# tgm-team/tgm

Measured on AMD Instinct MI355X. Metric: sampled-edges/sec (TGAT 2-hop k=20 recency sampler, tgbl-wiki synthetic), higher is better.
Workload: dtype int32/int64 indices + f32 feature rows (copied, no arithmetic)

## Files before the change

include/tgm_amd.h:

```cpp
#ifndef TGM_AMD_H
#define TGM_AMD_H

#include <stddef.h>
#include <stdint.h>

#ifdef __cplusplus
extern "C" {
#endif

#define TGMX_ABI_VERSION 7

#define TGMX_OK 0
#define TGMX_E_INVALID (-1)
#define TGMX_E_LAUNCH (-2)
#define TGMX_E_UNSUPPORTED (-3)

#define TGMX_ST_SEED_RANGE 1
#define TGMX_ST_SEED_TIME 2
#define TGMX_ST_EDGE_RANGE 4
#define TGMX_ST_SCRATCH 8
#define TGMX_ST_TS_BOUND 16

typedef void* tgmx_stream_t;
typedef void* tgmx_event_t;
// ... 74 lines not shown
  int64_t n, eid0;
  int32_t directed, key_wrap32;
  int32_t* scratch;
  int32_t* status;
  int32_t timed_hop;
  tgmx_event_t ev_start, ev_stop;
  int64_t ts_bound;
  int32_t neg_group, neg_low, neg_high;
  uint64_t neg_seed, neg_call;
  int32_t* neg_out;
  int64_t* neg_time_out;
  int32_t guard_seed_errors;
  int32_t sorted_ts;
  int32_t* out_valid[TGMX_MAX_HOPS];
  int32_t* out_valid_prev[TGMX_MAX_HOPS];
  int64_t neg_index0;
  int64_t* csr_cursor;
  int32_t csr_x_by_pos;
  int32_t* out_eid[TGMX_MAX_HOPS];
  struct tgmx_defer* defer;
  int32_t defer_ok;
} tgmx_recency_step_t;

int tgmx_recency_step(const tgmx_recency_step_t* step, tgmx_stream_t stream);
int tgmx_recency_step_plan(const tgmx_recency_step_t* step);

typedef struct tgmx_defer tgmx_defer_t;
tgmx_defer_t* tgmx_defer_create(int32_t num_nodes, int32_t B);
void tgmx_defer_destroy(tgmx_defer_t* d);
int tgmx_defer_pending(const tgmx_defer_t* d);
int64_t tgmx_defer_count(const tgmx_defer_t* d);
int tgmx_defer_flush(tgmx_defer_t* d, tgmx_stream_t stream);
int32_t tgmx_set_fused_rows(int32_t rows);

#define TGMX_SEED_SRC 0
#define TGMX_SEED_DST 1
#define TGMX_SEED_NEG 2
typedef struct tgmx_pipeline {
  const int32_t* src;
  const int32_t* dst;
  const int64_t* ts;
  const float* edge_x;
  int64_t num_edges;
  int32_t rank, world;
  int32_t n_roles;
  int32_t seed_role[TGMX_MAX_SEED_GROUPS];
  int32_t neg_low, neg_high;
  uint64_t neg_seed;
  int32_t update;
  int32_t reserved0;
  tgmx_recency_step_t step;
} tgmx_pipeline_t;

typedef struct tgmx_pipeline_out {
  int32_t* neg;
  int64_t* neg_time;
  int32_t* seed_nid0;
  int64_t* seed_ts0;
  int32_t* out_nid[TGMX_MAX_HOPS];
  int64_t* out_ts[TGMX_MAX_HOPS];
  float* out_x[TGMX_MAX_HOPS];
  int32_t timed_hop;
  tgmx_event_t ev_start, ev_stop;
  int32_t* out_valid[TGMX_MAX_HOPS];
  int32_t* out_valid_prev[TGMX_MAX_HOPS];
  int32_t* out_eid[TGMX_MAX_HOPS];
// ... 505 lines not shown
```

tgm_amd/_native.py:

```python
from __future__ import annotations

import ctypes
import os
from ctypes import c_char_p, c_int32, c_int64, c_size_t, c_void_p
from typing import Optional

import torch

from .exceptions import NativeLibraryError

_HERE = os.path.dirname(os.path.abspath(__file__))
LIB_PATH = os.path.join(_HERE, 'csrc', 'libtgm_amd.so')

_P = c_void_p
SIGNATURES = {
    'tgmx_version': (c_int32, []),
    'tgmx_abi_sizeof': (c_size_t, [c_int32]),
    'tgmx_last_error': (c_char_p, []),
    'tgmx_event_create': (c_int32, [ctypes.POINTER(c_void_p)]),
    'tgmx_event_destroy': (c_int32, [_P]),
    'tgmx_event_elapsed_ms': (c_int32, [_P, _P, ctypes.POINTER(ctypes.c_float)]),
    'tgmx_recency_lookup_csr': (
        c_int32,
        [_P, _P, _P, c_int32, _P, _P, c_int64, c_int32, c_int32, c_int64, c_int64, c_int32, c_int32, _P, _P, _P, _P, _P, _P, _P],
# ... 263 lines not shown


class Pipeline(ctypes.Structure):

    _fields_ = [
        ('src', c_void_p), ('dst', c_void_p), ('ts', c_void_p), ('edge_x', c_void_p), ('num_edges', c_int64),
        ('rank', c_int32), ('world', c_int32), ('n_roles', c_int32), ('seed_role', c_int32 * MAX_SEED_GROUPS),
        ('neg_low', c_int32), ('neg_high', c_int32), ('neg_seed', ctypes.c_uint64),
        ('update', c_int32), ('reserved0', c_int32), ('step', RecencyStep),
    ]


class PipelineOut(ctypes.Structure):

    _fields_ = [
        ('neg', c_void_p), ('neg_time', c_void_p), ('seed_nid0', c_void_p), ('seed_ts0', c_void_p),
        ('out_nid', c_void_p * MAX_HOPS), ('out_ts', c_void_p * MAX_HOPS), ('out_x', c_void_p * MAX_HOPS),
        ('timed_hop', c_int32), ('ev_start', c_void_p), ('ev_stop', c_void_p),
        ('out_valid', c_void_p * MAX_HOPS), ('out_valid_prev', c_void_p * MAX_HOPS), ('out_eid', c_void_p * MAX_HOPS),
    ]


ACCOUNTING_PARTIALS = 1024
SIGNATURES['tgmx_lookup_accounting'] = (c_int32, [_P, c_int64, _P, _P, c_int64, _P, _P])
SIGNATURES['tgmx_uniform_lookup_csr'] = (c_int32, [_P, _P, _P, c_int32, _P, c_int64, c_int32, c_int64, c_int32, c_int32, ctypes.c_uint64, ctypes.c_uint64,
                                                   _P, _P, _P, _P, _P])
SIGNATURES['tgmx_ring_update_scratch_bytes'] = (c_size_t, [c_int64, c_int32])
SIGNATURES['tgmx_defer_create'] = (c_void_p, [c_int32, c_int32])
SIGNATURES['tgmx_defer_destroy'] = (None, [_P])
SIGNATURES['tgmx_defer_pending'] = (c_int32, [_P])
SIGNATURES['tgmx_defer_count'] = (c_int64, [_P])
SIGNATURES['tgmx_defer_flush'] = (c_int32, [_P, _P])
SIGNATURES['tgmx_set_fused_rows'] = (c_int32, [c_int32])
SIGNATURES['tgmx_tgn_gru_gate_backward'] = (c_int32, [_P, _P, _P, _P, c_int32, c_int64, _P, _P, _P])
SIGNATURES['tgmx_tgn_aggregate_backward'] = (c_int32, [c_int64, _P, _P, _P, _P, _P, _P, c_int32, c_int32, _P, _P, c_int32, c_int32, _P, _P, _P])
SIGNATURES['tgmx_tconv_edge_attr_backward'] = (c_int32, [_P, _P, _P, _P, _P, _P, c_int32, c_int32, c_int64, _P, _P])
SIGNATURES['tgmx_tconv_attend_backward'] = (c_int32, [_P, _P, _P, _P, _P, _P, _P, _P, c_int64, c_int32, c_int32, ctypes.c_float, _P, _P, _P, _P, _P, _P, _P])
SIGNATURES['tgmx_group_ids'] = (c_int32, [_P, c_int32, _P, _P, _P, _P, _P, _P])
SIGNATURES['tgmx_group_ids_workspace_bytes'] = (c_size_t, [c_int64])
SIGNATURES['tgmx_group_ids_large'] = (c_int32, [_P, c_int64, _P, _P, _P, _P, _P, _P, c_size_t, _P])
SIGNATURES['tgmx_random_negatives'] = (c_int32, [c_int32, c_int32, c_int64, ctypes.c_uint64, ctypes.c_uint64, _P, _P, c_int64, _P, _P])
SIGNATURES['tgmx_random_negatives_at'] = (c_int32, [c_int32, c_int32, c_int64, ctypes.c_uint64, ctypes.c_uint64, c_int64, _P, _P, c_int64, _P, _P])
SIGNATURES['tgmx_unique_ids_workspace_bytes'] = (c_size_t, [c_int32])
SIGNATURES['tgmx_unique_ids'] = (c_int32, [_P, _P, c_int32, c_int32, _P, _P, _P, _P, _P])
SIGNATURES['tgmx_csr_build_workspace_bytes'] = (c_size_t, [c_int64, c_int32, c_int32])
SIGNATURES['tgmx_csr_build'] = (c_int32, [_P, _P, _P, c_int64, c_int32, _P, c_int64, c_int32, _P, _P, _P, c_size_t, _P, _P])
SIGNATURES['tgmx_recency_step'] = (c_int32, [ctypes.POINTER(RecencyStep), _P])
SIGNATURES['tgmx_recency_step_plan'] = (c_int32, [ctypes.POINTER(RecencyStep)])
SIGNATURES['tgmx_pipeline_step'] = (c_int32, [ctypes.POINTER(Pipeline), c_int64, c_int64, ctypes.c_uint64, ctypes.POINTER(PipelineOut), ctypes.POINTER(PipelinePost), _P])
SIGNATURES['tgmx_event_synchronize'] = (c_int32, [_P])
SIGNATURES['tgmx_event_create_sync'] = (c_int32, [ctypes.POINTER(c_void_p)])
SIGNATURES['tgmx_event_record'] = (c_int32, [_P, _P])
SIGNATURES['tgmx_stream_wait_event'] = (c_int32, [_P, _P])
SIGNATURES['tgmx_stream_handoff'] = (c_int32, [_P, _P, _P])
SIGNATURES['tgmx_worker_create'] = (c_int32, [ctypes.POINTER(c_void_p)])
SIGNATURES['tgmx_worker_destroy'] = (c_int32, [_P])
SIGNATURES['tgmx_worker_pipeline_step'] = (c_int32, [_P, ctypes.POINTER(Pipeline), c_int64, c_int64, ctypes.c_uint64, ctypes.POINTER(PipelineOut),
                                                     ctypes.POINTER(PipelinePost), _P, _P, _P, ctypes.POINTER(ctypes.c_uint64)])
SIGNATURES['tgmx_worker_wait'] = (c_int32, [_P, ctypes.c_uint64])
SIGNATURES['tgmx_slice'] = (c_int32, [_P, c_int64, c_int32, c_int64, c_int32, c_int64, c_int64, c_int64, ctypes.POINTER(c_int64), ctypes.POINTER(c_int64)])
SIGNATURES['tgmx_discretize_workspace_bytes'] = (c_size_t, [c_int64])
SIGNATURES['tgmx_discretize_keep'] = (c_int32, [_P, _P, _P, c_int64, ctypes.c_double, _P, _P, _P, _P, c_size_t, _P])
SIGNATURES['tgmx_tgn_memory_forward'] = (c_int32, [ctypes.POINTER(TgnMemoryFwd), _P])
SIGNATURES['tgmx_tconv_forward'] = (c_int32, [ctypes.POINTER(TconvFwd), _P])
SIGNATURES['tgmx_tgn_step'] = (c_int32, [ctypes.POINTER(TgnStep), _P])
SIGNATURES['tgmx_segment_sort_workspace_bytes'] = (c_size_t, [c_int64])
# ... 184 lines not shown
```

tgm_amd/csrc/recency.hip:

```cpp
#include <algorithm>
#include <atomic>
#include <cstdlib>
#include <cstring>
#include <string>
#include <vector>

#include <hip/hip_ext.h>
#include <rocprim/block/block_radix_sort.hpp>
#include <rocprim/block/block_scan.hpp>
#include <rocprim/device/device_radix_sort.hpp>
#include <rocprim/device/device_scan.hpp>
#include <rocprim/iterator/counting_iterator.hpp>
#include <rocprim/iterator/transform_iterator.hpp>

#include "common.h"

namespace tgmx {

struct __align__(16) Rec {
  int nbr;
  int eid;
  long long ts;
};
static_assert(sizeof(Rec) == sizeof(tgmx_adj_t), "record layout");
// ... 220 lines not shown

__device__ __forceinline__ int logical_wp(const int32_t* write_pos, const unsigned long long* phdr, unsigned pstamp, int n) {
  const int wp = write_pos[n];
  const unsigned long long h = phdr ? phdr[n] : 0ull;
  return (phdr && (unsigned)(h >> 32) == pstamp) ? (int)(unsigned)h : wp;
}

__device__ __forceinline__ void publish_wp(const UpdateArgs& a, int n, int w0, int kept) {
  unsigned long long* hp = &a.dhdr[n];
  unsigned long long cur = __hip_atomic_load(hp, __ATOMIC_RELAXED, __HIP_MEMORY_SCOPE_AGENT);
  for (;;) {
    const int base = (unsigned)(cur >> 32) == a.dstamp ? (int)(unsigned)cur : w0;
    const unsigned long long nv = ((unsigned long long)a.dstamp << 32) | (unsigned)fold_add(base, kept, a.B);
    const unsigned long long prev = atomicCAS(hp, cur, nv);
    if (prev == cur) break;
    cur = prev;
  }
}

template <int MAXM>
struct PlaceLds {
  int sn[MAXM];
  int len[MAXM];
  int h_key[2 * MAXM], h_maxp[2 * MAXM];
  long long red[kBlockThreads / kWave], red2[kBlockThreads / kWave];
  int wave_tot[kBlockThreads / kWave];
};
template <int MAXM>
struct SortLds {
  long long key[MAXM];
  int pay[MAXM];
};

template <typename T>
__device__ __forceinline__ void st_agent(T* p, T v) {
  __hip_atomic_store(p, v, __ATOMIC_RELAXED, __HIP_MEMORY_SCOPE_AGENT);
}
template <typename T>
__device__ __forceinline__ T ld_agent(const T* p) {
  return __hip_atomic_load(p, __ATOMIC_RELAXED, __HIP_MEMORY_SCOPE_AGENT);
}

template <int E, int MAXM, bool PRESORTED, bool DEFER, bool COH = false>
__device__ __forceinline__ void update_block_body(const UpdateArgs& a, PlaceLds<MAXM>& L, SortLds<PRESORTED ? 1 : MAXM>& S,
                                                  int part = 0, int parts = 1) {
  constexpr int H = 2 * MAXM;
  constexpr int HBITS = MAXM == 512 ? 10 : (MAXM == 1024 ? 11 : (MAXM == 2048 ? 12 : 13));
  static_assert((1 << HBITS) == H, "hash size");
  long long* s_key = S.key;
  int* s_pay = S.pay;
  int* s_sn = L.sn;
  int* s_len = L.len;
  int* h_key = L.h_key;
  int* h_maxp = L.h_maxp;
  long long* red = L.red;
  long long* red2 = L.red2;
  int* wave_tot = L.wave_tot;
  const int m = (int)a.m;
  const int tid = threadIdx.x, lane = tid & 63, wave = tid >> 6;
  const int nthr = blockDim.x, nwaves = nthr >> 6;
  const int P = nthr * E;
  const bool blocked = DEFER ? false : update_blocked(a);

  for (int x = tid; x < H; x += nthr) {
    h_key[x] = -1;
    h_maxp[x] = -1;
  }
  int pay[E], node[E], w[E];
  if constexpr (PRESORTED) {
#pragma unroll
    for (int r = 0; r < E; ++r) {
      const int p = tid * E + r;
      pay[r] = p;
      node[r] = -1;
      w[r] = 0;
      if (p < m) {
        pay[r] = COH ? ld_agent(&a.sorted_j[p]) : a.sorted_j[p];
        node[r] = COH ? ld_agent(&a.sorted_node[p]) : a.sorted_node[p];
        w[r] = COH ? ld_agent(&a.target[p]) : a.target[p];
      }
    }
  } else {
    static_assert(PRESORTED || E == 1, "the in-kernel sort holds one element per thread");
    long long mx = strided_max_ts(a.ts, a.n, tid, nthr), mn = strided_min_ts(a.ts, a.n, tid, nthr);
    for (int off = 32; off > 0; off >>= 1) {
      const long long o = __shfl_xor(mx, off), o2 = __shfl_xor(mn, off);
      mx = o > mx ? o : mx;
      mn = o2 < mn ? o2 : mn;
    }
    if (lane == 0) {
      red[wave] = mx;
      red2[wave] = mn;
    }
    __syncthreads();
    mx = red[0];
    mn = red2[0];
    for (int wv = 1; wv < nwaves; ++wv) {
      mx = red[wv] > mx ? red[wv] : mx;
      mn = red2[wv] < mn ? red2[wv] : mn;
    }
    const long long span = mx + 1;
    const bool packed = can_pack(a.key_wrap32, mn, mx);
// ... 69 lines not shown
    hs[r] = 0;
    cnt[r] = 0;
    if (p < m && node[r] >= 0 && (parts == 1 || node[r] % parts == part)) {
      cnt[r] = s_len[st[r]];
      const int pos = p - st[r];
      const int drop = cnt[r] > a.B ? cnt[r] - a.B : 0;
      if (pos >= drop) {
        const int t = node[r] * a.B + (w[r] + pos - drop) % a.B;
        unsigned h = ((unsigned)t * 2654435761u) >> (32 - HBITS);
        for (;;) {
          const int old = atomicCAS(&h_key[h], -1, t);
          if (old == -1 || old == t) break;
          h = (h + 1) & (H - 1);
        }
        atomicMax(&h_maxp[h], p);
        tgt[r] = t;
        hs[r] = (int)h;
      }
    }
  }
  __syncthreads();

#pragma unroll
  for (int r = 0; r < E; ++r) {
    const int p = tid * E + r;
    if (p >= m) continue;
    if (parts > 1 && (node[r] >= 0 ? node[r] % parts : 0) != part) continue;
    int win = -1, kept = 0;
    if (tgt[r] >= 0) {
      if (h_maxp[hs[r]] == p) {
        Rec rec;
        if constexpr (DEFER) {
          if (a.drec) {
            const long long* src = reinterpret_cast<const long long*>(&a.sorted_rec[p]);
            long long* dst = reinterpret_cast<long long*>(&a.drec[tgt[r]]);
            dst[0] = COH ? ld_agent(&src[0]) : src[0];
            dst[1] = COH ? ld_agent(&src[1]) : src[1];
            a.dslot[tgt[r]] = (int32_t)a.dstamp;
          }
        } else if constexpr (PRESORTED) {
          rec = a.sorted_rec[p];
        } else {
          int nd, nbr;
          long long t, i;
          update_entry(a, pay[r], nd, nbr, t, i);
          rec.nbr = nbr;
          rec.eid = a.eid0 >= 0 ? (int)(a.eid0 + i) : -1;
          rec.ts = t;
        }
        if constexpr (!DEFER) {
          if (!blocked) a.ring[tgt[r]] = rec;
        }
        win = blocked ? -1 : tgt[r];
      }
      if (p == st[r] + cnt[r] - 1) {
        kept = cnt[r] > a.B ? a.B : cnt[r];
        if constexpr (!DEFER) {
          if (!blocked) commit_write_pos(&a.write_pos[node[r]], kept, a.B);
        } else {
          if (a.dhdr) publish_wp(a, node[r], w[r], kept);
        }
      }
    }
    a.winner[p] = win;
    if constexpr (DEFER) a.target[p] = kept;
    if constexpr (!PRESORTED) a.sorted_j[p] = pay[r];
  }
}

template <int E, int MAXM, bool PRESORTED>
__global__ __launch_bounds__(kBlockThreads) void ring_update_block_kernel(const UpdateArgs a) {
  __shared__ PlaceLds<MAXM> L;
  __shared__ SortLds<PRESORTED ? 1 : MAXM> S;
  update_block_body<E, MAXM, PRESORTED, false>(a, L, S, (int)blockIdx.x, (int)gridDim.x);
}

template <int E, int MAXM>
__global__ __launch_bounds__(kBlockThreads) void ring_update_decide_kernel(const UpdateArgs a) {
  __shared__ PlaceLds<MAXM> L;
  __shared__ SortLds<1> S;
  update_block_body<E, MAXM, true, true>(a, L, S, (int)blockIdx.x, (int)gridDim.x);
}


struct ChunkSortLds {
  long long key[kChunk];
  int pay[kChunk];
  long long red[kChunk / kWave], red2[kChunk / kWave];
};

template <bool AGENT = false>
__device__ __forceinline__ void update_chunk_sort(const UpdateArgs& a, int chunk, ChunkSortLds& W) {
  long long* s_key = W.key;
  int* s_pay = W.pay;
  long long* red = W.red;
  long long* red2 = W.red2;
  const int tid = threadIdx.x, lane = tid & 63, wave = tid >> 6;
  long long mx = strided_max_ts(a.ts, a.n, tid, kChunk), mn = strided_min_ts(a.ts, a.n, tid, kChunk);
  for (int off = 32; off > 0; off >>= 1) {
// ... 167 lines not shown
  bool valid[NE];
#pragma unroll
  for (int q = 0; q < NE; ++q) {
    valid[q] = act[q] && node[q] >= 0 && node[q] < a.N && nbr[q] >= 0 && nbr[q] < a.N;
    w[q] = valid[q] ? logical_wp(a.write_pos, a.phdr, a.pstamp, node[q]) : 0;
  }
#pragma unroll
  for (int q = 0; q < NE; ++q) {
    if (!act[q]) continue;
    int rank = tid;
#pragma unroll
    for (int o = 0; o < NC; ++o) rank += pos[q][o] >= 0 ? pos[q][o] : 0;
    if (!valid[q]) atomicOr(a.status, TGMX_ST_EDGE_RANGE);
    Rec rec;
    rec.nbr = nbr[q];
    rec.eid = a.eid0 >= 0 ? (int)(a.eid0 + i[q]) : -1;
    rec.ts = t[q];
    if constexpr (COH) {
      st_agent(&a.sorted_j[rank], pay[q]);
      st_agent(&a.sorted_node[rank], valid[q] ? node[q] : -1);
      st_agent(&a.target[rank], w[q]);
      long long* rd = reinterpret_cast<long long*>(&a.sorted_rec[rank]);
      st_agent(&rd[0], *reinterpret_cast<const long long*>(&rec));
      st_agent(&rd[1], rec.ts);
    } else {
      a.sorted_j[rank] = pay[q];
      a.sorted_node[rank] = valid[q] ? node[q] : -1;
      a.target[rank] = w[q];
      a.sorted_rec[rank] = rec;
    }
  }
}

constexpr int kSideSort = 1, kSideMerge = 2, kSidePlace = 3, kSideAll = 4, kSideSortMerge = 5, kSidePlaceOnly = 6, kSideSortMergePlace = 7, kSideMergePlace = 8;

__device__ __forceinline__ bool rider_barrier(int32_t* bar, int parts) {
  __syncthreads();
  bool ok = true;
  if (threadIdx.x == 0) {
    const int gen = __hip_atomic_load(&bar[1], __ATOMIC_RELAXED, __HIP_MEMORY_SCOPE_AGENT);
    const int prev = __hip_atomic_fetch_add(&bar[0], 1, __ATOMIC_RELAXED, __HIP_MEMORY_SCOPE_AGENT);
    if (prev == parts - 1) {
      __hip_atomic_store(&bar[0], 0, __ATOMIC_RELAXED, __HIP_MEMORY_SCOPE_AGENT);
      __builtin_amdgcn_s_waitcnt(0);
      __hip_atomic_fetch_add(&bar[1], 1, __ATOMIC_RELAXED, __HIP_MEMORY_SCOPE_AGENT);
    } else {
      int spins = 0;
      while (__hip_atomic_load(&bar[1], __ATOMIC_RELAXED, __HIP_MEMORY_SCOPE_AGENT) == gen) {
        __builtin_amdgcn_s_sleep(8);
        if (++spins > (1 << 19)) {
          ok = false;
          break;
        }
      }
    }
  }
  __syncthreads();
  return ok;
}
constexpr int kRidePlaceMaxM = 1024;

__device__ __forceinline__ void commit_position(const UpdateArgs& a, long long p) {
  const int row = a.winner[p];
  if (lane_id() == 0) {
    const int kept = a.target[p];
    if (row >= 0) a.ring[row] = a.sorted_rec[p];
    if (kept > 0) {
      const int n = a.sorted_node[p];
      if (a.dhdr) a.write_pos[n] = (int)(unsigned)a.dhdr[n];
      else commit_write_pos(&a.write_pos[n], kept, a.B);
    }
  }
  if (row < 0 || a.D == 0) return;
  const long long j = a.sorted_j[p];
  const long long i = j >= a.n ? j - a.n : j;
  float* __restrict__ o = a.ring_x + (long long)row * a.D;
  if (a.edge_x) {
    const float* __restrict__ x = a.edge_x + i * a.D;
    for (int c = lane_id(); c < a.D; c += kWave) o[c] = x[c];
  } else {
    for (int c = lane_id(); c < a.D; c += kWave) o[c] = 0.f;
  }
}

__device__ __forceinline__ void commit_block(const UpdateArgs& c, unsigned cb) {
  const long long p = (long long)cb * (blockDim.x >> 6) + (threadIdx.x >> 6);
  if (p < c.m) commit_position(c, p);
}

template <int PCAP>
union RiderLds {
  ChunkSortLds sort;
  SampleLds smp;
  PlaceLds<PCAP> place;
};
template <>
union RiderLds<0> {
  ChunkSortLds sort;
  SampleLds smp;
};

template <int PCAP = kRidePlaceMaxM>
__device__ __forceinline__ void update_side_work(const UpdateArgs& u, int stage, int block) {
  __shared__ RiderLds<PCAP> W;
  if (stage == kSideSort) {
    update_chunk_sort(u, block, W.sort);
  } else if (stage == kSideMerge) {
    update_merge_riding<1, kBlockMaxM / kChunk>(u, block, W.smp);
  } else if (stage == kSideSortMerge) {
    update_chunk_sort<true>(u, block, W.sort);
    if (!rider_barrier(u.barrier, (int)((u.m + kChunk - 1) / kChunk)) && threadIdx.x == 0) atomicOr(u.status, TGMX_ST_SCRATCH);
    update_merge_riding<1, kBlockMaxM / kChunk>(u, block, W.smp);
  } else if constexpr (PCAP > 0) {
    constexpr int NCH = PCAP / kChunk;
    if (stage == kSideSortMergePlace) {
      const int chunks = (int)((u.m + kChunk - 1) / kChunk);
      __shared__ int last_out;
      update_chunk_sort<true>(u, block, W.sort);
      if (!rider_barrier(u.barrier, chunks) && threadIdx.x == 0) atomicOr(u.status, TGMX_ST_SCRATCH);
      update_merge_riding<1, NCH, true>(u, block, W.smp);
      __syncthreads();
      if (threadIdx.x == 0) {
        const int prev = __hip_atomic_fetch_add(&u.barrier[5], 1, __ATOMIC_RELAXED, __HIP_MEMORY_SCOPE_AGENT);
        last_out = prev == chunks - 1;
        if (last_out) __hip_atomic_store(&u.barrier[5], 0, __ATOMIC_RELAXED, __HIP_MEMORY_SCOPE_AGENT);
      }
      __syncthreads();
      if (!last_out) return;
      SortLds<1> none;
      update_block_body<NCH, PCAP, true, true, true>(u, W.place, none);
      return;
    }
    if (stage == kSideMergePlace) {
      const int chunks = (int)((u.m + kChunk - 1) / kChunk);
      __shared__ int last_mp;
      update_merge_riding<1, NCH, true>(u, block, W.smp);
      __syncthreads();
      if (threadIdx.x == 0) {
        const int prev = __hip_atomic_fetch_add(&u.barrier[5], 1, __ATOMIC_RELAXED, __HIP_MEMORY_SCOPE_AGENT);
        last_mp = prev == chunks - 1;
        if (last_mp) __hip_atomic_store(&u.barrier[5], 0, __ATOMIC_RELAXED, __HIP_MEMORY_SCOPE_AGENT);
      }
      __syncthreads();
      if (!last_mp) return;
      SortLds<1> none;
      update_block_body<NCH, PCAP, true, true, true>(u, W.place, none);
      return;
    }
    if (stage == kSideAll) {
      const int chunks = (int)((u.m + kChunk - 1) / kChunk);
#pragma unroll 1
      for (int c = 0; c < NCH; ++c) {
        if (c < chunks) update_chunk_sort(u, c, W.sort);
        __syncthreads();
      }
    }
    if (stage != kSidePlaceOnly) {
      update_merge_riding<NCH, NCH>(u, 0, W.smp);
      __syncthreads();
    }
    SortLds<1> none;
    update_block_body<NCH, PCAP, true, true>(u, W.place, none);
  }
}


template <int GL>
__device__ __forceinline__ long long group_prefix_count(const Rec* recs, long long a, long long z, long long bound, int gl, int sub) {
  constexpr unsigned long long kMask = GL == 64 ? ~0ull : ((1ull << GL) - 1);
  long long lo = a, hi = z;
  while (__any(hi - lo > GL)) {
    const bool busy = hi - lo > GL;
    const long long len = hi - lo;
    const long long stride = (len + GL - 1) / GL;
    long long idx = lo + (long long)(gl + 1) * stride - 1;
    if (idx > hi - 1) idx = hi - 1;
    const bool less = busy && (long long)recs[idx].eid < bound;
    const int c = __popcll((__ballot(less) >> (sub * GL)) & kMask);
    if (busy) {
      long long nlo = lo, nhi = hi;
      if (c > 0) {
// ... 186 lines not shown
__device__ __forceinline__ void gather_rows(const LookupArgs& a, long long s, int k, int lane, const int* lds_eid, float* out_x, int first_slot) {
  using V = typename VecOf<VEC>::type;
  const V* __restrict__ X = reinterpret_cast<const V*>(a.edge_x);
  const int lim = a.pstore ? a.N * a.B : 0x7fffffff;
  const V* __restrict__ P = a.pstore ? reinterpret_cast<const V*>(a.pstore) : X;
  V* __restrict__ O = reinterpret_cast<V*>(out_x + s * (long long)k * a.D);
  const int total = k * a.row_vecs;
  constexpr int U = 8;
  for (int f0 = first_slot * a.row_vecs + lane; f0 < total; f0 += kWave * U) {
    const V* ptr[U];
    bool has[U];
#pragma unroll
    for (int u = 0; u < U; ++u) {
      const int f = f0 + u * kWave;
      const int fc = f < total ? f : f0;
      const int slot = (int)a.dv.div_nb((uint32_t)fc);
      const int col = fc - slot * a.row_vecs;
      const int e = lds_eid[slot];
      has[u] = e >= 0;
      const bool st = e >= lim;
      ptr[u] = (st ? P : X) + (has[u] ? (long long)(st ? e - lim : e) * a.row_vecs + col : 0);
    }
    V v[U];
#pragma unroll
    for (int u = 0; u < U; ++u) v[u] = *ptr[u];
#pragma unroll
    for (int u = 0; u < U; ++u) {
      const int f = f0 + u * kWave;
      if (f < total) O[f] = has[u] ? v[u] : zero_vec<V>();
    }
  }
}

template <bool RING, int VEC, bool SMALL>
__device__ __forceinline__ void lookup_seed(const LookupArgs& a, long long s, int n, long long q, int k, int lane, int* lds_eid,
                                            int32_t* out_nid, int64_t* out_ts, float* out_x, int32_t* out_valid, int32_t* out_valid_prev,
                                            int32_t* out_eid = nullptr) {
  const bool live = n >= 0 && n < a.N;
  int v_new = 0;
  if (SMALL) {
    const SmallPick o = small_pick<RING>(a, n, q, k, live, lane);
    if (lane < k) {
      out_nid[s * k + lane] = o.nbr;
      out_ts[s * k + lane] = o.ts;
      if (out_eid) out_eid[s * k + lane] = o.eid;
      lds_eid[lane] = o.src;
    }
    const unsigned long long m = __ballot(lane < k && o.has);
    v_new = m ? k - __builtin_ctzll(m) : 0;
  } else {
    const int B = a.B;
    const Window w = find_window<RING>(a, n, live, lane);
    int cnt = 0;
    for (int top = w.wlen; top > 0 && cnt == 0; top -= kWave) {
      const int lo = top > kWave ? top - kWave : 0;
      const int i = lo + lane;
      bool ok = false;
      if (i < top) {
        const Rec r = a.recs[slot_of<RING>(w, B, i)];
        ok = r.nbr >= 0 && r.ts < q;
      }
      const unsigned long long m = __ballot(ok);
      if (m) cnt = lo + 64 - __clzll((long long)m);
    }
    for (int c = lane; c < k; c += kWave) {
      const int i = cnt - k + c;
      Rec r;
      r.nbr = -1; r.eid = 0; r.ts = 0;
      if (i >= 0) r = a.recs[slot_of<RING>(w, B, i)];
      const bool has = r.nbr >= 0;
      out_nid[s * k + c] = has ? r.nbr : -1;
      out_ts[s * k + c] = has ? r.ts : 0;
      if (out_eid) out_eid[s * k + c] = has ? r.eid : -1;
      lds_eid[c] = has ? ((RING || a.x_by_pos) ? (int)slot_of<RING>(w, B, i) : r.eid) : -1;
      if (has && k - c > v_new) v_new = k - c;
    }
    for (int o = 32; o > 0; o >>= 1) {
      const int other = __shfl_xor(v_new, o);
      v_new = other > v_new ? other : v_new;
    }
  }
  if (a.D == 0 || out_x == nullptr) return;
  int first_slot = 0;
  if (out_valid) {
    const int v_old = out_valid[s];
    first_slot = k - (v_old > v_new ? v_old : v_new);
    if (lane == 0) {
      out_valid[s] = v_new;
      if (out_valid_prev) out_valid_prev[s] = v_old;
    }
  }
  __builtin_amdgcn_wave_barrier();
  gather_rows<VEC>(a, s, k, lane, lds_eid, out_x, first_slot);
  __builtin_amdgcn_wave_barrier();
}

template <bool RING, int VEC, bool SMALL, bool RIDE>
__global__ __launch_bounds__(256) void recency_lookup_kernel(const LookupArgs a, const UpdateArgs u) {
  extern __shared__ __attribute__((aligned(16))) int lds_eid_all[];
  unsigned bid = blockIdx.x, nblk = gridDim.x;
  if constexpr (RING && RIDE) {
    if (bid < a.side_blocks) {
      update_side_work(u, a.side_stage, (int)bid);
      return;
    }
    bid -= a.side_blocks;
    nblk -= a.side_blocks;
  }
  const int lane = lane_id();
  const int wave_in_block = threadIdx.x >> 6;
  int* lds_eid = lds_eid_all + wave_in_block * a.k;
  const long long waves_total = (long long)nblk * (blockDim.x >> 6);
  for (long long s = (long long)bid * (blockDim.x >> 6) + wave_in_block; s < a.S; s += waves_total) {
    int n;
    long long q;
    fetch_seed(a, s, lane, true, n, q);
    check_seed(a, n, q, a.allow_pad, lane);
    lookup_seed<RING, VEC, SMALL>(a, s, n, q, a.k, lane, lds_eid, a.out_nid, a.out_ts, a.out_x, a.out_valid, a.out_valid_prev, a.out_eid);
  }
}

constexpr int kFusedTsWords = 8;
constexpr int kFusedRowsDefault = 0;
enum FusedTsRole : long long { kTsRider = 1, kTsCommit = 2, kTsHop0 = 3, kTsHop1 = 4 };
__device__ __forceinline__ long long ts_after(int v) {
  asm volatile("" ::"v"(v));
  return (long long)wall_clock64();
}

template <bool RING>
__device__ __forceinline__ SmallPick fused_row_pick(const LookupArgs& a, const PickLoads& L, int n, long long q, bool live, int lane) {
  if constexpr (RING) return pick_finish(a, L, n, q, a.k1, live, lane);
  else return small_pick<false>(a, n, q, a.k1, live, lane);
}

template <bool RING, int VEC, int PCAP = kRidePlaceMaxM, bool ROWS = false, bool TS = false>
__global__ __launch_bounds__(256) void recency_lookup_fused01_kernel(const LookupArgs a, const UpdateArgs u, const UpdateArgs c) {
  extern __shared__ __attribute__((aligned(16))) int lds_eid_all[];
  unsigned bid = blockIdx.x, nblk = gridDim.x;
  const int lane = lane_id();
  const int wave_in_block = threadIdx.x >> 6;
  long long* ts_rec = TS ? a.ts + ((long long)blockIdx.x * (blockDim.x >> 6) + wave_in_block) * kFusedTsWords : nullptr;
  const long long t_start = TS ? (long long)wall_clock64() : 0;
  if constexpr (RING) {
    if (bid < a.side_blocks) {
      update_side_work<PCAP>(u, a.side_stage, (int)bid);
      if (TS && lane == 0) {
        ts_rec[0] = t_start;
        ts_rec[1] = (long long)wall_clock64();
        ts_rec[2] = kTsRider;
      }
      return;
    }
    bid -= a.side_blocks;
    if (bid < a.commit_blocks) {
      commit_block(c, bid);
      if (TS && lane == 0) {
        ts_rec[0] = t_start;
        ts_rec[1] = (long long)wall_clock64();
        ts_rec[2] = kTsCommit;
      }
      return;
    }
    bid -= a.commit_blocks;
    nblk -= a.side_blocks + a.commit_blocks;
  }
  const int k0 = a.k, k1 = a.k1;
  int* lds_eid = lds_eid_all + wave_in_block * (k0 > k1 ? k0 : k1);
  const long long waves_total = (long long)nblk * (blockDim.x >> 6);
  const long long S0 = a.S;
  const int G = ROWS ? a.fused_rows : 0;
  const int runs = G > 0 ? (k0 + G - 1) / G : k0;
  long long role = 0, t_seed = 0, t_index = 0, t_gather = 0;
  for (long long w = (long long)bid * (blockDim.x >> 6) + wave_in_block; w < S0 + S0 * runs; w += waves_total) {
    int n;
    long long q;
    if (w < S0) {
      role = kTsHop0;
      fetch_seed(a, w, lane, true, n, q);
      check_seed(a, n, q, 0, lane);
      lookup_seed<RING, VEC, true>(a, w, n, q, k0, lane, lds_eid, a.out_nid, a.out_ts, a.out_x, a.out_valid, a.out_valid_prev, a.out_eid);
    } else if (!ROWS) {
      role = kTsHop1;
      const long long idx = w - S0;
      const long long s0 = idx / k0;
      const int j = (int)(idx - s0 * k0);
      int n0;
      long long q0;
      fetch_seed(a, s0, lane, false, n0, q0);
      const SmallPick o = small_pick<RING>(a, n0, q0, k0, n0 >= 0 && n0 < a.N, lane);
      n = __shfl(o.nbr, j);
      q = __shfl(o.ts, j);
      lookup_seed<RING, VEC, true>(a, idx, n, q, k1, lane, lds_eid, a.out_nid1, a.out_ts1, a.out_x1, a.out_valid1, a.out_valid_prev1, a.out_eid1);
    } else {
      const long long run = w - S0;
      const long long s0 = run / runs;
      const int j0 = (int)(run - s0 * runs) * G;
      const int rows = k0 - j0 < G ? k0 - j0 : G;
      const long long base = s0 * k0 + j0;
      const bool feats = a.D > 0 && a.out_x1 != nullptr;
      const int v_old_run = (feats && a.out_valid1 && lane < rows) ? a.out_valid1[base + lane] : 0;
      int n0;
      long long q0;
      fetch_seed(a, s0, lane, false, n0, q0);
      const SmallPick o0 = small_pick<RING>(a, n0, q0, k0, n0 >= 0 && n0 < a.N, lane);
      n = __shfl(o0.nbr, j0);
      q = __shfl(o0.ts, j0);
      bool live = n >= 0 && n < a.N;
      if (TS) {
        role = kTsHop1 | ((long long)rows << 8);
        t_seed = ts_after(n);
      }
      PickLoads L = RING ? pick_issue(a, n, live, lane) : PickLoads{};
      for (int r = 0; r < rows; ++r) {
        const long long s = base + r;
        const long long t0 = TS ? (long long)wall_clock64() : 0;
        const SmallPick o = fused_row_pick<RING>(a, L, n, q, live, lane);
        if (lane < k1) {
          a.out_nid1[s * k1 + lane] = o.nbr;
          a.out_ts1[s * k1 + lane] = o.ts;
          if (a.out_eid1) a.out_eid1[s * k1 + lane] = o.eid;
          lds_eid[lane] = o.src;
        }
        const unsigned long long m = __ballot(lane < k1 && o.has);
        const int v_new = m ? k1 - __builtin_ctzll(m) : 0;
        if (TS) {
// ... 829 lines not shown
  static unsigned long long launches = 0;
  const long long waves = (long long)blocks_total * waves_per_block;
  std::vector<long long> h((size_t)(8 + waves * kFusedTsWords));
  if (hipStreamSynchronize(stream) != hipSuccess ||
      hipMemcpy(h.data() + 8, a.ts, (size_t)waves * kFusedTsWords * sizeof(long long), hipMemcpyDeviceToHost) != hipSuccess) {
    set_error("recency_lookup_fused01: reading the timestamps failed");
    return TGMX_E_LAUNCH;
  }
  int dev = 0, khz = 0;
  (void)hipGetDevice(&dev);
  (void)hipDeviceGetAttribute(&khz, hipDeviceAttributeWallClockRate, dev);
  const long long hdr[8] = {0x54474d5854530001ll, waves, (long long)a.side_blocks, (long long)a.commit_blocks, a.S, a.k, a.fused_rows, khz};
  std::copy(hdr, hdr + 8, h.begin());
  const std::string path = std::string(fused_ts_path()) + "." + std::to_string(launches++ % 16);
  if (FILE* f = fopen(path.c_str(), "wb")) {
    fwrite(h.data(), sizeof(long long), h.size(), f);
    fclose(f);
  }
  return TGMX_OK;
}

static std::atomic<int> g_fused_rows{-1};

static int fused_rows_per_wave(int k0) {
  int g = g_fused_rows.load(std::memory_order_relaxed);
  if (g < 0) {
    const char* e = getenv("TGMX_FUSED_ROWS");
    g = (e && *e && atoi(e) >= 0) ? atoi(e) : kFusedRowsDefault;
    g_fused_rows.store(g, std::memory_order_relaxed);
  }
  return g > k0 ? k0 : g;
}

template <bool RING>
static int launch_fused01(LookupArgs a, hipStream_t stream, hipEvent_t ev_start, hipEvent_t ev_stop, const UpdateArgs* side,
                          int side_stage, unsigned side_blocks, const UpdateArgs* commit = nullptr) {
  const UpdateArgs u = side ? *side : UpdateArgs{};
  const UpdateArgs c = (RING && commit) ? *commit : UpdateArgs{};
  a.side_blocks = (RING && side) ? side_blocks : 0;
  a.side_stage = side_stage;
  a.commit_blocks = (RING && commit) ? (unsigned)((c.m + 3) / 4) : 0u;
  a.fused_rows = fused_rows_per_wave(a.k);
  const int kmax = a.k > a.k1 ? a.k : a.k1;
  const int vec = prepare_lookup(a, a.out_x1, kmax);
  if (vec < 0) return vec;
  const int waves_per_block = 4;
  const long long runs = a.fused_rows > 0 ? (a.k + a.fused_rows - 1) / a.fused_rows : a.k;
  const long long waves = a.S + a.S * runs;
  long long blocks = (waves + waves_per_block - 1) / waves_per_block;
  if (blocks > (1 << 20)) blocks = 1 << 20;
  const dim3 grid((unsigned)blocks + a.side_blocks + a.commit_blocks), block(waves_per_block * kWave);
  const size_t lds = (size_t)waves_per_block * kmax * sizeof(int);
  const int pcap = !(RING && side) ? 1024 : ((side_stage != kSideAll && side_stage != kSideSortMergePlace) ? 0 : (u.m <= 512 ? 512 : 1024));
  if (RING && vec == 4 && pcap == 512 && fused_ts_path()) {
    static long long* ts_buf = nullptr;
    static size_t ts_cap = 0;
    const size_t need = (size_t)grid.x * waves_per_block * kFusedTsWords * sizeof(long long);
    if (need > ts_cap) {
      if (ts_buf) (void)hipFree(ts_buf);
      ts_buf = nullptr;
      if (hipMalloc(&ts_buf, need) != hipSuccess) {
        set_error("recency_lookup_fused01: no memory for the timestamps");
        return TGMX_E_LAUNCH;
      }
      ts_cap = need;
    }
    a.ts = ts_buf;
    (void)hipMemsetAsync(a.ts, 0, need, stream);
    if (a.fused_rows > 0) TGMX_LAUNCH_TIMED((recency_lookup_fused01_kernel<true, 4, 512, true, true>), grid, block, lds, stream, ev_start, ev_stop, a, u, c);
    else TGMX_LAUNCH_TIMED((recency_lookup_fused01_kernel<true, 4, 512, false, true>), grid, block, lds, stream, ev_start, ev_stop, a, u, c);
    TGMX_CHECK_LAUNCH("recency_lookup_fused01");
    return fused_ts_dump(a, stream, grid.x, waves_per_block);
  }
#define TGMX_FUSED(ROWS_)                                                                                                                            \
  do {                                                                                                                                               \
    if (vec == 4 && pcap == 512) TGMX_LAUNCH_TIMED((recency_lookup_fused01_kernel<RING, 4, RING ? 512 : 1024, ROWS_>), grid, block, lds, stream, ev_start, ev_stop, a, u, c); \
    else if (vec == 4 && pcap == 0) TGMX_LAUNCH_TIMED((recency_lookup_fused01_kernel<RING, 4, RING ? 0 : 1024, ROWS_>), grid, block, lds, stream, ev_start, ev_stop, a, u, c); \
    else if (vec == 4) TGMX_LAUNCH_TIMED((recency_lookup_fused01_kernel<RING, 4, kRidePlaceMaxM, ROWS_>), grid, block, lds, stream, ev_start, ev_stop, a, u, c);            \
    else if (vec == 2) TGMX_LAUNCH_TIMED((recency_lookup_fused01_kernel<RING, 2, kRidePlaceMaxM, ROWS_>), grid, block, lds, stream, ev_start, ev_stop, a, u, c);            \
    else TGMX_LAUNCH_TIMED((recency_lookup_fused01_kernel<RING, 1, kRidePlaceMaxM, ROWS_>), grid, block, lds, stream, ev_start, ev_stop, a, u, c);                          \
  } while (0)
  if (a.fused_rows > 0) TGMX_FUSED(true);
  else TGMX_FUSED(false);
#undef TGMX_FUSED
  TGMX_CHECK_LAUNCH("recency_lookup_fused01");
  return TGMX_OK;
// ... 719 lines not shown
}

extern "C" void tgmx_defer_destroy(tgmx_defer_t* d) {
  if (d && d->mem) (void)hipFree(d->mem);
  delete d;
}

static int defer_buffers(tgmx_defer* d, hipStream_t st) {
  if (d->mem) return TGMX_OK;
  auto up = [](size_t x) { return (x + 255) & ~(size_t)255; };
  const size_t nb = (size_t)d->N * d->B;
  const size_t half = up(tgmx_ring_update_scratch_bytes(kRidePlaceMaxM, 1));
  const size_t o_scr = up((size_t)16 * d->N), o_slot = o_scr + 2 * half, o_rec = up(o_slot + 8 * nb), total = o_rec + 32 * nb;
  void* mem = nullptr;
  if (hipMalloc(&mem, total) != hipSuccess) {
    set_error("recency_step: cannot allocate %zu bytes for the deferred commit", total);
    return TGMX_E_LAUNCH;
  }
  (void)hipMemsetAsync(mem, 0, o_rec, st);
  char* base = static_cast<char*>(mem);
  d->mem = mem;
  for (int q = 0; q < 2; ++q) {
    d->hdr[q] = reinterpret_cast<unsigned long long*>(base) + (size_t)q * d->N;
    d->scratch[q] = reinterpret_cast<int32_t*>(base + o_scr + q * half);
    d->slot[q] = reinterpret_cast<int32_t*>(base + o_slot) + q * nb;
    d->rec[q] = reinterpret_cast<Rec*>(base + o_rec) + q * nb;
  }
  return TGMX_OK;
}

extern "C" int tgmx_defer_pending(const tgmx_defer_t* d) { return d && d->pending ? 1 : 0; }

extern "C" int64_t tgmx_defer_count(const tgmx_defer_t* d) { return d ? d->deferred : 0; }
extern "C" int32_t tgmx_set_fused_rows(int32_t rows) {
  const int old = fused_rows_per_wave(1 << 30);
  g_fused_rows.store(rows < 0 ? -1 : rows, std::memory_order_relaxed);
  return old;
}

extern "C" int tgmx_defer_flush(tgmx_defer_t* d, tgmx_stream_t stream) {
  TGMX_REQUIRE(d, "defer_flush: null state");
  if (!d->pending) return TGMX_OK;
  d->pending = false;
  hipLaunchKernelGGL(ring_update_feat_kernel<true>, dim3((unsigned)((d->pend.m + 3) / 4)), dim3(256), 0, (hipStream_t)stream, d->pend);
  TGMX_CHECK_LAUNCH("defer_flush");
  return TGMX_OK;
}

static bool getenv_no_ride() {
  static const bool no_ride = getenv("TGMX_NO_RIDE") != nullptr;
  return no_ride;
}


static bool plan_fuse01(const tgmx_recency_step_t* s, long long S0) {
  static const bool no_fuse = getenv("TGMX_NO_FUSE") != nullptr;
  if (no_fuse || s->n_hops < 2 || S0 <= 0 || s->B > kWave || s->k[0] <= 0 || s->k[1] <= 0) return false;
  if (s->indptr != nullptr && (long long)s->k[1] * s->D * 4 < 4096) return false;
  static const bool fuse_by_id = !(getenv("TGMX_FUSE_BY_ID") && atoi(getenv("TGMX_FUSE_BY_ID")) == 0);
  const bool by_id = s->out_eid[1] != nullptr && s->out_x[1] == nullptr;
  if (s->indptr == nullptr && !(by_id && fuse_by_id)) {
    LookupArgs a{};
    a.B = s->B; a.D = s->D; a.edge_x = s->ring_x; a.out_x = s->out_x[0];
    if (prepare_lookup(a, s->out_x[1], s->k[1]) < 0) return false;
    if (packed_group_lanes(a, s->k[1], true) < 64) return false;
  }
// ... 221 lines not shown
```

Baseline: 9.458 billion.

## Add LDS-resident sort-and-place path for single rider block; hoist valid-span load

Adds a rider stage that sorts the update batch entirely in LDS (bitonic sort per chunk plus merge-rank across chunks) and feeds the deferred placement directly from LDS. This avoids writing and re-reading sorted records through global memory between stages. Separately, the old valid-span read is hoisted ahead of the seed fetch so its latency overlaps. The LDS path is gated by an env/setter flag that defaults off, so the default run only gets the hoisted load. The enlarged LDS union may reduce occupancy of the fused kernel.

Result: no change. 9.436 billion (-0.2%).

```diff
diff --git a/include/tgm_amd.h b/include/tgm_amd.h
--- a/include/tgm_amd.h
+++ b/include/tgm_amd.h
@@ -130,6 +130,7 @@
 int64_t tgmx_defer_count(const tgmx_defer_t* d);
 int tgmx_defer_flush(tgmx_defer_t* d, tgmx_stream_t stream);
 int32_t tgmx_set_fused_rows(int32_t rows);
+int32_t tgmx_set_rider_lds(int32_t on);
 
 #define TGMX_SEED_SRC 0
 #define TGMX_SEED_DST 1
diff --git a/tgm_amd/_native.py b/tgm_amd/_native.py
--- a/tgm_amd/_native.py
+++ b/tgm_amd/_native.py
@@ -319,6 +319,7 @@
 SIGNATURES['tgmx_defer_count'] = (c_int64, [_P])
 SIGNATURES['tgmx_defer_flush'] = (c_int32, [_P, _P])
 SIGNATURES['tgmx_set_fused_rows'] = (c_int32, [c_int32])
+SIGNATURES['tgmx_set_rider_lds'] = (c_int32, [c_int32])
 SIGNATURES['tgmx_tgn_gru_gate_backward'] = (c_int32, [_P, _P, _P, _P, c_int32, c_int64, _P, _P, _P])
 SIGNATURES['tgmx_tgn_aggregate_backward'] = (c_int32, [c_int64, _P, _P, _P, _P, _P, _P, c_int32, c_int32, _P, _P, c_int32, c_int32, _P, _P, _P])
 SIGNATURES['tgmx_tconv_edge_attr_backward'] = (c_int32, [_P, _P, _P, _P, _P, _P, c_int32, c_int32, c_int64, _P, _P])
diff --git a/tgm_amd/csrc/recency.hip b/tgm_amd/csrc/recency.hip
--- a/tgm_amd/csrc/recency.hip
+++ b/tgm_amd/csrc/recency.hip
@@ -276,6 +276,16 @@
   int pay[MAXM];
 };
 
+constexpr int kRiderLdsM = 2 * kChunk;
+struct SortedLds {
+  long long key[kRiderLdsM];
+  long long ts[kRiderLdsM];
+  int pay[kRiderLdsM];
+  int node[kRiderLdsM], nbr[kRiderLdsM];
+  int spay[kRiderLdsM];
+  long long red[kChunk / kWave], red2[kChunk / kWave];
+};
+
 template <typename T>
 __device__ __forceinline__ void st_agent(T* p, T v) {
   __hip_atomic_store(p, v, __ATOMIC_RELAXED, __HIP_MEMORY_SCOPE_AGENT);
@@ -285,9 +295,10 @@
   return __hip_atomic_load(p, __ATOMIC_RELAXED, __HIP_MEMORY_SCOPE_AGENT);
 }
 
-template <int E, int MAXM, bool PRESORTED, bool DEFER, bool COH = false>
+template <int E, int MAXM, bool PRESORTED, bool DEFER, bool COH = false, bool FROMLDS = false>
 __device__ __forceinline__ void update_block_body(const UpdateArgs& a, PlaceLds<MAXM>& L, SortLds<PRESORTED ? 1 : MAXM>& S,
-                                                  int part = 0, int parts = 1) {
+                                                  int part = 0, int parts = 1, const SortedLds* F = nullptr) {
+  static_assert(!FROMLDS || (PRESORTED && DEFER && !COH), "the LDS-fed placement is the deferred one of a single rider");
   constexpr int H = 2 * MAXM;
   constexpr int HBITS = MAXM == 512 ? 10 : (MAXM == 1024 ? 11 : (MAXM == 2048 ? 12 : 13));
   static_assert((1 << HBITS) == H, "hash size");
@@ -306,12 +317,37 @@
   const int P = nthr * E;
   const bool blocked = DEFER ? false : update_blocked(a);
 
+  int pay[E], node[E], w[E];
+  [[maybe_unused]] Rec lrec[FROMLDS ? E : 1];
+  if constexpr (FROMLDS) {
+#pragma unroll
+    for (int r = 0; r < E; ++r) {
+      const int p = tid * E + r;
+      pay[r] = p;
+      node[r] = -1;
+      w[r] = 0;
+      lrec[r].nbr = -1; lrec[r].eid = -1; lrec[r].ts = 0;
+      if (p < m) {
+        const int j = F->spay[p];
+        const int nd = F->node[j], nb = F->nbr[j];
+        const bool valid = nd >= 0 && nd < a.N && nb >= 0 && nb < a.N;
+        if (!valid) atomicOr(a.status, TGMX_ST_EDGE_RANGE);
+        pay[r] = j;
+        node[r] = valid ? nd : -1;
+        w[r] = valid ? logical_wp(a.write_pos, a.phdr, a.pstamp, nd) : 0;
+        lrec[r].nbr = nb;
+        lrec[r].eid = a.eid0 >= 0 ? (int)(a.eid0 + (j >= a.n ? j - a.n : j)) : -1;
+        lrec[r].ts = F->ts[j];
+      }
+    }
+    __syncthreads();
+  }
   for (int x = tid; x < H; x += nthr) {
     h_key[x] = -1;
     h_maxp[x] = -1;
   }
-  int pay[E], node[E], w[E];
-  if constexpr (PRESORTED) {
+  if constexpr (FROMLDS) {
+  } else if constexpr (PRESORTED) {
 #pragma unroll
     for (int r = 0; r < E; ++r) {
       const int p = tid * E + r;
@@ -447,10 +483,14 @@
         Rec rec;
         if constexpr (DEFER) {
           if (a.drec) {
-            const long long* src = reinterpret_cast<const long long*>(&a.sorted_rec[p]);
-            long long* dst = reinterpret_cast<long long*>(&a.drec[tgt[r]]);
-            dst[0] = COH ? ld_agent(&src[0]) : src[0];
-            dst[1] = COH ? ld_agent(&src[1]) : src[1];
+            if constexpr (FROMLDS) {
+              a.drec[tgt[r]] = lrec[r];
+            } else {
+              const long long* src = reinterpret_cast<const long long*>(&a.sorted_rec[p]);
+              long long* dst = reinterpret_cast<long long*>(&a.drec[tgt[r]]);
+              dst[0] = COH ? ld_agent(&src[0]) : src[0];
+              dst[1] = COH ? ld_agent(&src[1]) : src[1];
+            }
             a.dslot[tgt[r]] = (int32_t)a.dstamp;
           }
         } else if constexpr (PRESORTED) {
@@ -480,6 +520,11 @@
     a.winner[p] = win;
     if constexpr (DEFER) a.target[p] = kept;
     if constexpr (!PRESORTED) a.sorted_j[p] = pay[r];
+    if constexpr (FROMLDS) {
+      a.sorted_j[p] = pay[r];
+      a.sorted_node[p] = node[r];
+      a.sorted_rec[p] = lrec[r];
+    }
   }
 }
 
@@ -713,7 +758,89 @@
   }
 }
 
-constexpr int kSideSort = 1, kSideMerge = 2, kSidePlace = 3, kSideAll = 4, kSideSortMerge = 5, kSidePlaceOnly = 6, kSideSortMergePlace = 7, kSideMergePlace = 8;
+__device__ __forceinline__ void rider_sort_lds(const UpdateArgs& a, SortedLds& F) {
+  constexpr int NCH = kRiderLdsM / kChunk;
+  const int m = (int)a.m;
+  const int tid = threadIdx.x, lane = tid & 63, wave = tid >> 6;
+  const int chunks = (m + kChunk - 1) / kChunk;
+  long long mx = strided_max_ts(a.ts, a.n, tid, kChunk), mn = strided_min_ts(a.ts, a.n, tid, kChunk);
+  int node[NCH], nbr[NCH];
+  long long t[NCH];
+#pragma unroll
+  for (int q = 0; q < NCH; ++q) {
+    const int j = q * kChunk + tid;
+    long long i;
+    node[q] = nbr[q] = -1;
+    t[q] = 0;
+    if (j < m) update_entry(a, j, node[q], nbr[q], t[q], i);
+  }
+  for (int off = 32; off > 0; off >>= 1) {
+    const long long o = __shfl_xor(mx, off), o2 = __shfl_xor(mn, off);
+    mx = o > mx ? o : mx;
+    mn = o2 < mn ? o2 : mn;
+  }
+  if (lane == 0) {
+    F.red[wave] = mx;
+    F.red2[wave] = mn;
+  }
+  __syncthreads();
+  mx = F.red[0];
+  mn = F.red2[0];
+  for (int w = 1; w < kChunk / kWave; ++w) {
+    mx = F.red[w] > mx ? F.red[w] : mx;
+    mn = F.red2[w] < mn ? F.red2[w] : mn;
+  }
+  const long long span = mx + 1;
+  const bool packed = can_pack(a.key_wrap32, mn, mx);
+  long long key[NCH];
+  int pay[NCH];
+#pragma unroll
+  for (int q = 0; q < NCH; ++q) {
+    const int j = q * kChunk + tid;
+    key[q] = 0x7fffffffffffffffLL;
+    pay[q] = j;
+    if (j < m) {
+      key[q] = update_key(node[q], t[q], span, a.key_wrap32);
+      if (packed) key[q] = packed_key(key[q], j);
+      F.node[j] = node[q];
+      F.nbr[j] = nbr[q];
+      F.ts[j] = t[q];
+    }
+  }
+#pragma unroll
+  for (int q = 0; q < NCH; ++q) {
+    if (q < chunks) {
+      if (packed) bitonic_sort_one<true>(key[q], pay[q], F.key, F.pay, tid, kChunk);
+      else bitonic_sort_one<false>(key[q], pay[q], F.key, F.pay, tid, kChunk);
+    }
+  }
+#pragma unroll
+  for (int q = 0; q < NCH; ++q) {
+    F.key[q * kChunk + tid] = key[q];
+    F.pay[q * kChunk + tid] = pay[q];
+  }
+  __syncthreads();
+#pragma unroll
+  for (int q = 0; q < NCH; ++q) {
+    if (q * kChunk + tid >= m) continue;
+    int rank = tid;
+#pragma unroll
+    for (int o = 0; o < NCH; ++o) {
+      if (o == q || o >= chunks) continue;
+      int lo = 0, hi = m - o * kChunk < kChunk ? m - o * kChunk : kChunk;
+      while (lo < hi) {
+        const int mid = (lo + hi) >> 1;
+        if (pair_after(key[q], pay[q], F.key[o * kChunk + mid], F.pay[o * kChunk + mid])) lo = mid + 1;
+        else hi = mid;
+      }
+      rank += lo;
+    }
+    F.spay[rank] = pay[q];
+  }
+  __syncthreads();
+}
+
+constexpr int kSideSort = 1, kSideMerge = 2, kSidePlace = 3, kSideAll = 4, kSideSortMerge = 5, kSidePlaceOnly = 6, kSideSortMergePlace = 7, kSideMergePlace = 8, kSideAllLds = 9;
 
 __device__ __forceinline__ bool rider_barrier(int32_t* bar, int parts) {
   __syncthreads();
@@ -774,6 +901,7 @@
   ChunkSortLds sort;
   SampleLds smp;
   PlaceLds<PCAP> place;
+  SortedLds sorted;
 };
 template <>
 union RiderLds<0> {
@@ -828,6 +956,14 @@
       update_block_body<NCH, PCAP, true, true, true>(u, W.place, none);
       return;
     }
+    if constexpr (PCAP == kRiderLdsM) {
+      if (stage == kSideAllLds) {
+        rider_sort_lds(u, W.sorted);
+        SortLds<1> none;
+        update_block_body<NCH, PCAP, true, true, false, true>(u, W.place, none, 0, 1, &W.sorted);
+        return;
+      }
+    }
     if (stage == kSideAll) {
       const int chunks = (int)((u.m + kChunk - 1) / kChunk);
 #pragma unroll 1
@@ -1080,10 +1216,14 @@
   }
 }
 
+__device__ __forceinline__ int load_span(const LookupArgs& a, const float* out_x, const int32_t* out_valid, long long s) {
+  return (a.D > 0 && out_x != nullptr && out_valid != nullptr) ? out_valid[s] : 0;
+}
+
 template <bool RING, int VEC, bool SMALL>
 __device__ __forceinline__ void lookup_seed(const LookupArgs& a, long long s, int n, long long q, int k, int lane, int* lds_eid,
                                             int32_t* out_nid, int64_t* out_ts, float* out_x, int32_t* out_valid, int32_t* out_valid_prev,
-                                            int32_t* out_eid = nullptr) {
+                                            int v_old, int32_t* out_eid = nullptr) {
   const bool live = n >= 0 && n < a.N;
   int v_new = 0;
   if (SMALL) {
@@ -1131,7 +1271,6 @@
   if (a.D == 0 || out_x == nullptr) return;
   int first_slot = 0;
   if (out_valid) {
-    const int v_old = out_valid[s];
     first_slot = k - (v_old > v_new ? v_old : v_new);
     if (lane == 0) {
       out_valid[s] = v_new;
@@ -1162,9 +1301,10 @@
   for (long long s = (long long)bid * (blockDim.x >> 6) + wave_in_block; s < a.S; s += waves_total) {
     int n;
     long long q;
+    const int v_old = load_span(a, a.out_x, a.out_valid, s);
     fetch_seed(a, s, lane, true, n, q);
     check_seed(a, n, q, a.allow_pad, lane);
-    lookup_seed<RING, VEC, SMALL>(a, s, n, q, a.k, lane, lds_eid, a.out_nid, a.out_ts, a.out_x, a.out_valid, a.out_valid_prev, a.out_eid);
+    lookup_seed<RING, VEC, SMALL>(a, s, n, q, a.k, lane, lds_eid, a.out_nid, a.out_ts, a.out_x, a.out_valid, a.out_valid_prev, v_old, a.out_eid);
   }
 }
 
@@ -1225,12 +1365,14 @@
     long long q;
     if (w < S0) {
       role = kTsHop0;
+      const int v_old = load_span(a, a.out_x, a.out_valid, w);
       fetch_seed(a, w, lane, true, n, q);
       check_seed(a, n, q, 0, lane);
-      lookup_seed<RING, VEC, true>(a, w, n, q, k0, lane, lds_eid, a.out_nid, a.out_ts, a.out_x, a.out_valid, a.out_valid_prev, a.out_eid);
+      lookup_seed<RING, VEC, true>(a, w, n, q, k0, lane, lds_eid, a.out_nid, a.out_ts, a.out_x, a.out_valid, a.out_valid_prev, v_old, a.out_eid);
     } else if (!ROWS) {
       role = kTsHop1;
       const long long idx = w - S0;
+      const int v_old = load_span(a, a.out_x1, a.out_valid1, idx);
       const long long s0 = idx / k0;
       const int j = (int)(idx - s0 * k0);
       int n0;
@@ -1239,7 +1381,7 @@
       const SmallPick o = small_pick<RING>(a, n0, q0, k0, n0 >= 0 && n0 < a.N, lane);
       n = __shfl(o.nbr, j);
       q = __shfl(o.ts, j);
-      lookup_seed<RING, VEC, true>(a, idx, n, q, k1, lane, lds_eid, a.out_nid1, a.out_ts1, a.out_x1, a.out_valid1, a.out_valid_prev1, a.out_eid1);
+      lookup_seed<RING, VEC, true>(a, idx, n, q, k1, lane, lds_eid, a.out_nid1, a.out_ts1, a.out_x1, a.out_valid1, a.out_valid_prev1, v_old, a.out_eid1);
     } else {
       const long long run = w - S0;
       const long long s0 = run / runs;
@@ -2135,6 +2277,19 @@
   return g > k0 ? k0 : g;
 }
 
+constexpr int kRiderLdsDefault = 0;
+static std::atomic<int> g_rider_lds{-1};
+
+static int rider_lds_on() {
+  int g = g_rider_lds.load(std::memory_order_relaxed);
+  if (g < 0) {
+    const char* e = getenv("TGMX_RIDER_LDS");
+    g = (e && *e && atoi(e) >= 0) ? (atoi(e) != 0) : kRiderLdsDefault;
+    g_rider_lds.store(g, std::memory_order_relaxed);
+  }
+  return g;
+}
+
 template <bool RING>
 static int launch_fused01(LookupArgs a, hipStream_t stream, hipEvent_t ev_start, hipEvent_t ev_stop, const UpdateArgs* side,
                           int side_stage, unsigned side_blocks, const UpdateArgs* commit = nullptr) {
@@ -2155,6 +2310,7 @@
   const dim3 grid((unsigned)blocks + a.side_blocks + a.commit_blocks), block(waves_per_block * kWave);
   const size_t lds = (size_t)waves_per_block * kmax * sizeof(int);
   const int pcap = !(RING && side) ? 1024 : ((side_stage != kSideAll && side_stage != kSideSortMergePlace) ? 0 : (u.m <= 512 ? 512 : 1024));
+  if (RING && side && side_stage == kSideAll && vec == 4 && pcap == 512 && a.side_blocks == 1 && rider_lds_on()) a.side_stage = kSideAllLds;
   if (RING && vec == 4 && pcap == 512 && fused_ts_path()) {
     static long long* ts_buf = nullptr;
     static size_t ts_cap = 0;
@@ -2940,6 +3096,12 @@
 extern "C" int tgmx_defer_pending(const tgmx_defer_t* d) { return d && d->pending ? 1 : 0; }
 
 extern "C" int64_t tgmx_defer_count(const tgmx_defer_t* d) { return d ? d->deferred : 0; }
+extern "C" int32_t tgmx_set_rider_lds(int32_t on) {
+  const int old = rider_lds_on();
+  g_rider_lds.store(on < 0 ? -1 : (on != 0), std::memory_order_relaxed);
+  return old;
+}
+
 extern "C" int32_t tgmx_set_fused_rows(int32_t rows) {
   const int old = fused_rows_per_wave(1 << 30);
   g_fused_rows.store(rows < 0 ? -1 : rows, std::memory_order_relaxed);
```
